# fperezgamonal/flownet2-tf

Hardware: AMD Instinct MI355X
Metric: forward pairs/sec at 512x384 (FlowNet2) (higher is better)
Workload: dtype f16x2 (split fp16 hi+lo operands, 3 fp16 MFMAs per product, fp32 accumulate); 1 GPU; FlowNet2 forward, batch=4 synthetic 512x384 pairs per GPU, seeded synthetic weights; pairs_per_gpu=4, parallelism=dp1 (no collective)

## Files before the change

flownet2-tf_amd/csrc/conv2.hip:

```cpp
#include "conv_common.h"

#include <type_traits>
#include <algorithm>
#include <utility>

#ifndef FN2_X2_ORDER
#define FN2_X2_ORDER 0
#endif
#ifndef FN2_CONV_ABLATE
#define FN2_CONV_ABLATE 0
#endif
#ifndef FN2_SETPRIO
#define FN2_SETPRIO 1
#endif

namespace fn2 {

typedef __attribute__((address_space(3))) void* lptr_t;

constexpr unsigned kOobOffset = 0x80000000u;

typedef int v4i_t __attribute__((ext_vector_type(4)));
typedef unsigned u32x4_t __attribute__((ext_vector_type(4)));

// ... 606 lines not shown
      const int m = m0 + wp * TPN * 32 + b * 16 + r16;
      if (m >= p.M) continue;
      const int n = m / (p.OH * p.OW);
      const int rem = m - n * (p.OH * p.OW);
      const int oy = rem / p.OW, ox = rem - oy * p.OW;
      const size_t opix = ((size_t)n * p.out_H + (oy * osc + oy_off)) * p.out_W + (ox * osc + ox_off);
      OutT* po = out16 + opix * p.out_cs + p.out_c0;
#pragma unroll
      for (int a = 0; a < TCN * 2; ++a) {
        const int co = c0 + wc * TCN * 32 + (a >> 1) * 32 + 16 * (g16 & 1) + 8 * (a & 1) + 4 * (g16 >> 1);
        if (slab != nullptr) {
          if (co < p.ws_cs)
            *reinterpret_cast<float4*>(slab + opix * p.ws_cs + co) =
                make_float4(acc16[a][b][0], acc16[a][b][1], acc16[a][b][2], acc16[a][b][3]);
          continue;
        }
        float v[4];
#pragma unroll
        for (int j = 0; j < 4; ++j) {
          float x = acc16[a][b][j] * p.out_scale + ((p.bias != nullptr && co + j < p.Cout) ? p.bias[co + j] : 0.f);
          if constexpr (sizeof(OutT) == 4) {
            if (p.accum && co + j < p.Cout) x += load_elem<OutT>(po + co + j);
            if (co + j < p.Cout) x = act_grad<OutT>(p, out16, po + co + j, co + j, x);
          }
          if (p.act == FN2_ACT_LEAKY) x = leaky(x);
          v[j] = x;
        }
        if (p.vec_ok && co + 3 < p.Cout) store_vec<OutT, 4>(po + co, v);
        else
#pragma unroll
          for (int j = 0; j < 4; ++j)
            if (co + j < p.Cout) store_elem<OutT>(po + co + j, v[j]);
      }
    }
    return;
  }

  OutT* out = reinterpret_cast<OutT*>(p.out);
  constexpr int WCOLS = TCN * 32, RS = WCOLS + 4, WROWS = 32 * TPN;
  constexpr int WTW = WROWS * RS + WROWS;
  constexpr bool kLdsT = (KG > 1 ? 4 : 2) * WTW * 4 <= KG * ROWS * 128;
  if constexpr (FEED && !kLdsT) { if (feeder) return; }
  float* const tl = reinterpret_cast<float*>(KG > 1 ? ep1 : (wave < 2 ? lds0_all : ep1)) + (KG > 1 ? wave : (wave & 1)) * WTW;
  constexpr int CPR = WCOLS / 4, RPI = 64 / CPR;
  static_assert(!SLAB || WREG, "SLAB is a specialisation of the WREG instantiations");
  if ((SLAB || !WREG) && p.splitk > 1) {
    float* slab = p.ws + (size_t)split * p.N * p.out_H * p.out_W * p.ws_cs;
    if constexpr (kLdsT) {
      if constexpr (STAGES >= 3) __syncthreads();
      if constexpr (FEED) { if (feeder) return; }
      int* rowoff = reinterpret_cast<int*>(tl + WROWS * RS);
#pragma unroll
      for (int tp = 0; tp < TPN; ++tp) {
        const int m = m0 + wp * TPN * 32 + tp * 32 + fr;
        const int mm = m < p.M ? m : 0;
        const int n = mm / (p.OH * p.OW);
        const int rem = mm - n * (p.OH * p.OW);
        const int oy = rem / p.OW, ox = rem - oy * p.OW;
        if (fh == 0) rowoff[tp * 32 + fr] = m < p.M ? (int)((((size_t)n * p.out_H + (oy * osc + oy_off)) * p.out_W + (ox * osc + ox_off)) * p.ws_cs) : -1;
#pragma unroll
        for (int tc = 0; tc < TCN; ++tc)
#pragma unroll
          for (int q = 0; q < 4; ++q)
            *reinterpret_cast<float4*>(tl + (tp * 32 + fr) * RS + tc * 32 + fh * 16 + q * 4) =
                make_float4(acc[tc][tp][4 * q], acc[tc][tp][4 * q + 1], acc[tc][tp][4 * q + 2], acc[tc][tp][4 * q + 3]);
      }
      const int rr = lane / CPR, ch = lane - rr * CPR;
      const int co = c0 + wc * WCOLS + ch * 4;
#pragma unroll
      for (int i = 0; i < WROWS / RPI; ++i) {
        const int row = i * RPI + rr;
        const float4 v = *reinterpret_cast<const float4*>(tl + row * RS + ch * 4);
        const int off = rowoff[row];
        if (off >= 0 && co < p.ws_cs) *reinterpret_cast<float4*>(slab + (size_t)off + co) = v;
      }
      return;
    }
#pragma unroll
    for (int tp = 0; tp < TPN; ++tp) {
      const int m = m0 + wp * TPN * 32 + tp * 32 + fr;
      if (m >= p.M) continue;
      const int n = m / (p.OH * p.OW);
      const int rem = m - n * (p.OH * p.OW);
      const int oy = rem / p.OW, ox = rem - oy * p.OW;
      float* po = slab + (((size_t)n * p.out_H + (oy * osc + oy_off)) * p.out_W + (ox * osc + ox_off)) * p.ws_cs;
#pragma unroll
      for (int tc = 0; tc < TCN; ++tc)
#pragma unroll
        for (int q = 0; q < 4; ++q) {
          const int co = c0 + wc * TCN * 32 + tc * 32 + fh * 16 + q * 4;
          if (co < p.ws_cs)
            *reinterpret_cast<float4*>(po + co) = make_float4(acc[tc][tp][4 * q], acc[tc][tp][4 * q + 1],
                                                              acc[tc][tp][4 * q + 2], acc[tc][tp][4 * q + 3]);
        }
    }
    return;
  }
  if constexpr (SLAB) return;
  const bool vec16 = (p.out_cs % 8 == 0) && (p.out_c0 % 8 == 0);
  const bool wide = kLdsT && sizeof(OutT) == 4 && vec16 && c0 + wc * WCOLS + WCOLS <= p.Cout && !(p.dbg & 4194304);
  int* const rowoff = reinterpret_cast<int*>(tl + WROWS * RS);
  if constexpr (STAGES >= 3 && kLdsT) __syncthreads();
  if constexpr (FEED) { if (feeder) return; }
#pragma unroll
  for (int tc = 0; tc < TCN; ++tc) {
    const int cout_base = c0 + wc * TCN * 32 + tc * 32 + fh * 16;
    float bias[16];
#pragma unroll
    for (int q = 0; q < 16; ++q) bias[q] = (p.bias != nullptr && cout_base + q < p.Cout) ? p.bias[cout_base + q] : 0.f;
#pragma unroll
    for (int tp = 0; tp < TPN; ++tp) {
      const int m = m0 + wp * TPN * 32 + tp * 32 + fr;
      if (wide && tc == 0 && fh == 0) rowoff[tp * 32 + fr] = m < p.M ? 0 : -1;
      if (m >= p.M) continue;
      const int n = m / (p.OH * p.OW);
      const int rem = m - n * (p.OH * p.OW);
      const int oy = rem / p.OW, ox = rem - oy * p.OW;
      const size_t opix = (((size_t)n * p.out_H + (oy * osc + oy_off)) * p.out_W + (ox * osc + ox_off));
      OutT* po = out + opix * p.out_cs + p.out_c0 + cout_base;
      float v[16];
#pragma unroll
      for (int q = 0; q < 16; ++q) v[q] = acc[tc][tp][q] * p.out_scale + bias[q];
      accum_act_grad16<OutT>(p, out, po, cout_base, vec16 && cout_base + 15 < p.Cout, v);
      if (p.act == FN2_ACT_LEAKY) {
#pragma unroll
        for (int q = 0; q < 16; ++q) v[q] = leaky(v[q]);
      }
      if (wide) {
        if (tc == 0 && fh == 0) rowoff[tp * 32 + fr] = (int)opix;
        store16<OutT>(reinterpret_cast<OutT*>(tl + (tp * 32 + fr) * RS + tc * 32 + fh * 16), v);
      } else if (vec16 && cout_base + 15 < p.Cout) {
        store16<OutT>(po, v);
      } else {
#pragma unroll
        for (int q = 0; q < 16; ++q)
          if (cout_base + q < p.Cout) store_elem<OutT>(po + q, v[q]);
      }
    }
  }
  if (wide) {
    const int rr = lane / CPR, ch = lane - rr * CPR;
    OutT* ob = out + p.out_c0 + c0 + wc * WCOLS + ch * 4;
#pragma unroll
    for (int i = 0; i < WROWS / RPI; ++i) {
      const int row = i * RPI + rr;
      const uint4 v = *reinterpret_cast<const uint4*>(tl + row * RS + ch * 4);
      const int opix = rowoff[row];
      if (opix >= 0) *reinterpret_cast<uint4*>(ob + (size_t)opix * p.out_cs) = v;
    }
  }
#endif
}

template <typename OutT, int WC, int WP, int TCN, int TPN, int KW>
__global__ void __launch_bounds__(256) conv_halo_kernel(const ConvArgs p) {
#if defined(__HIP_DEVICE_COMPILE__)
  using T = x2_t;
  constexpr int ESZ = 4;
  constexpr int BC = WC * TCN * 32, BP = WP * TPN * 32;
  static_assert(WC * WP == 4, "4 waves per block");
  constexpr int NWI = BC / 32;
  constexpr int BROWS = BP + 8;
  constexpr int NBP = BROWS / 8;
  constexpr int NBW = (NBP + 3) / 4;
  __shared__ uint4 ldsA[2][BC * 8];
  __shared__ uint4 ldsB[2][BROWS * 8];

  const int tid = threadIdx.x, lane = tid & 63;
  const int wave = __builtin_amdgcn_readfirstlane(tid >> 6);
  const int wc = wave / WP, wp = wave % WP;

  int pad_y = p.pad, pad_x = p.pad, oy_off = 0, ox_off = 0, osc = 1;
  const T* wgt = reinterpret_cast<const T*>(p.wgt);
  const int phase = blockIdx.z;
  const unsigned wrow_bytes = (unsigned)p.ksteps * 128u;
  if (p.merged) {
    pad_y = phase ? p.ph_pad1 : p.ph_pad0; pad_x = 1; oy_off = phase; ox_off = 0; osc = 2;
    wgt += (size_t)phase * p.cout_pad * (wrow_bytes / ESZ);
  } else if (p.deconv) {
    const int a = phase >> 1, b = phase & 1;
    pad_y = a ? p.ph_pad1 : p.ph_pad0; pad_x = b ? p.ph_pad1 : p.ph_pad0; oy_off = a; ox_off = b; osc = 2;
    wgt += (size_t)phase * p.cout_pad * (wrow_bytes / ESZ);
  }
  int bx = blockIdx.x, by = blockIdx.y;
  {
    const int NT = gridDim.x * gridDim.y, L = blockIdx.x + gridDim.x * blockIdx.y;
    const int xcd = L & 7, chunk = NT >> 3, rem = NT & 7;
    const int Lp = xcd * chunk + min(xcd, rem) + (L >> 3);
    bx = Lp / (int)gridDim.y;
    by = Lp - bx * (int)gridDim.y;
  }
  const int m0 = bx * BP, c0 = by * BC;
  const int tn = m0 / (p.OH * p.OW);
  const int trem = m0 - tn * (p.OH * p.OW);
  const int toy = trem / p.OW, tox = trem - toy * p.OW;
  const int iy_base = toy - pad_y, ix_base = tox - pad_x;

  const v4i_t rsrc_w = make_rsrc(wgt, (int)(p.cout_pad * wrow_bytes));
  const v4i_t rsrc_x = make_rsrc(p.in, p.in_bytes);
  const int lrow = lane >> 3, lphys = lane & 7;
  unsigned woff[NWI];
#pragma unroll
  for (int j = 0; j < NWI; ++j) {
    const int row = wave * (BC / 4) + j * 8 + lrow;
    woff[j] = (unsigned)(c0 + row) * wrow_bytes + (unsigned)((lphys ^ ((row >> 1) & 7)) * 16);
  }
  int boff[NBW];
  bool bok[NBW];
#pragma unroll
  for (int j = 0; j < NBW; ++j) {
    const int q = wave + 4 * j;
    const int e = q * 8 + lrow;
    const int ix = ix_base + e;
    bok[j] = q < NBP && e < BP + KW - 1 && ix >= 0 && ix < p.W;
    boff[j] = (((tn * p.H + iy_base) * p.W + ix) * p.in_cs + p.in_c0) * ESZ + (lphys ^ ((e >> 1) & 7)) * 16;
  }
  const int spt = p.cin_chunks >> 3;
  const int nsup = spt * p.KH;
  auto issue_B = [&](int sup, uint4* lds) {
    const int sc = sup / p.KH, ky = sup - sc * p.KH;
    const bool yok = (unsigned)(iy_base + ky) < (unsigned)p.H;
    const int toff = (ky * p.W * p.in_cs) * ESZ + sc * 128;
#pragma unroll
    for (int j = 0; j < NBW; ++j) {
      const int q = wave + 4 * j;
      if (q < NBP) dma16(rsrc_x, &lds[q * 64], (bok[j] && yok) ? (unsigned)(boff[j] + toff) : kOobOffset, 0);
    }
  };
  auto issue_A = [&](int sup, int kx, uint4* lds) {
    const int sc = sup / p.KH, ky = sup - sc * p.KH;
    const int soff = ((ky * KW + kx) * spt + sc) * 128;
#pragma unroll
    for (int j = 0; j < NWI; ++j) dma16(rsrc_w, &lds[(wave * (BC / 4) + j * 8) * 8], woff[j], soff);
  };

  const int fr = lane & 31, fh = lane >> 5, fsw = (fr >> 1) & 7;
  f32x16 acc[TCN][TPN];
#pragma unroll
  for (int tc = 0; tc < TCN; ++tc)
#pragma unroll
    for (int tp = 0; tp < TPN; ++tp)
#pragma unroll
      for (int q = 0; q < 16; ++q) acc[tc][tp][q] = 0.f;

  auto compute = [&](const uint4* la, const uint4* lb, int kx) {
#if FN2_SETPRIO
    __builtin_amdgcn_s_setprio(1);
#endif
    const uint4* A = &la[(wc * TCN * 32 + fr) * 8];
#pragma unroll
    for (int q = 0; q < 2; ++q) {
      const int chh = (4 * q + 2 * fh) ^ fsw, chl = (4 * q + 2 * fh + 1) ^ fsw;
      uint4 ah[TCN], al[TCN], bh[TPN], bl[TPN];
#pragma unroll
      for (int t = 0; t < TCN; ++t) { ah[t] = A[t * 32 * 8 + chh]; al[t] = A[t * 32 * 8 + chl]; }
#pragma unroll
      for (int t = 0; t < TPN; ++t) {
        const int rb = wp * TPN * 32 + t * 32 + fr + kx, sw = (rb >> 1) & 7;
        bh[t] = lb[rb * 8 + ((4 * q + 2 * fh) ^ sw)];
        bl[t] = lb[rb * 8 + ((4 * q + 2 * fh + 1) ^ sw)];
      }
#pragma unroll
      for (int tc = 0; tc < TCN; ++tc)
#pragma unroll
        for (int tp = 0; tp < TPN; ++tp) {
          acc[tc][tp] = mfma_32x32x16<f16_t>(al[tc], bh[tp], acc[tc][tp]);
          acc[tc][tp] = mfma_32x32x16<f16_t>(ah[tc], bl[tp], acc[tc][tp]);
          acc[tc][tp] = mfma_32x32x16<f16_t>(ah[tc], bh[tp], acc[tc][tp]);
        }
    }
#if FN2_SETPRIO
    __builtin_amdgcn_s_setprio(0);
#endif
  };

  issue_B(0, ldsB[0]);
  issue_A(0, 0, ldsA[0]);
  asm volatile("s_waitcnt vmcnt(0)" ::: "memory");
  __syncthreads();
  int abuf = 0;
  for (int sup = 0; sup < nsup; ++sup) {
#pragma unroll
    for (int kx = 0; kx < KW; ++kx) {
      if (kx + 1 < KW) issue_A(sup, kx + 1, ldsA[abuf ^ 1]);
      else if (sup + 1 < nsup) issue_A(sup + 1, 0, ldsA[abuf ^ 1]);
      if (kx == 0 && sup + 1 < nsup) issue_B(sup + 1, ldsB[(sup + 1) & 1]);
      compute(ldsA[abuf], ldsB[sup & 1], kx);
      asm volatile("s_waitcnt vmcnt(0)" ::: "memory");
      __syncthreads();
      abuf ^= 1;
    }
  }

  OutT* out = reinterpret_cast<OutT*>(p.out);
  const bool vec16 = (p.out_cs % 8 == 0) && (p.out_c0 % 8 == 0);
  constexpr int ERS = 36;
  static_assert(sizeof(ldsA) >= 4 * 32 * ERS * 4 || sizeof(ldsB) >= 4 * 32 * ERS * 4, "epilogue tiles fit a stage array");
  float* const etl = reinterpret_cast<float*>(sizeof(ldsA) >= 4 * 32 * ERS * 4 ? &ldsA[0][0] : &ldsB[0][0]) + wave * (32 * ERS);
#pragma unroll
  for (int tc = 0; tc < TCN; ++tc) {
    int cout_base = c0 + wc * TCN * 32 + tc * 32 + fh * 16;
    int bsel = 0;
    if (p.merged) { bsel = cout_base / p.Cout; cout_base -= bsel * p.Cout; if (bsel > 1) continue; }
    float bias[16];
#pragma unroll
    for (int q = 0; q < 16; ++q) bias[q] = (p.bias != nullptr && cout_base + q < p.Cout) ? p.bias[cout_base + q] : 0.f;
#pragma unroll
    for (int tp = 0; tp < TPN; ++tp) {
      const int ox = tox + wp * TPN * 32 + tp * 32 + fr;
      OutT* po = out + (((size_t)tn * p.out_H + (toy * osc + oy_off)) * p.out_W + (ox * osc + ox_off + bsel)) * p.out_cs +
                 p.out_c0 + cout_base;
      float v[16];
#pragma unroll
      for (int q = 0; q < 16; ++q) v[q] = acc[tc][tp][q] * p.out_scale + bias[q];
      accum_act_grad16<OutT>(p, out, po, cout_base, vec16 && cout_base + 15 < p.Cout, v);
      if (p.act == FN2_ACT_LEAKY) {
#pragma unroll
        for (int q = 0; q < 16; ++q) v[q] = leaky(v[q]);
      }
      if (sizeof(OutT) == 4 && vec16 && !p.merged && c0 + wc * TCN * 32 + tc * 32 + 32 <= p.Cout && !(p.dbg & 4194304)) {
        store16<OutT>(reinterpret_cast<OutT*>(etl + fr * ERS + fh * 16), v);
        const int rr = lane >> 3, ch = lane & 7;
        const int ox0 = tox + wp * TPN * 32 + tp * 32;
        OutT* ob = out + (((size_t)tn * p.out_H + (toy * osc + oy_off)) * p.out_W + (ox0 * osc + ox_off)) * p.out_cs +
                   p.out_c0 + c0 + wc * TCN * 32 + tc * 32 + ch * 4;
#pragma unroll
        for (int i = 0; i < 4; ++i) {
          const int row = i * 8 + rr;
          *reinterpret_cast<uint4*>(ob + (size_t)row * osc * p.out_cs) = *reinterpret_cast<const uint4*>(etl + row * ERS + ch * 4);
        }
      } else if (vec16 && cout_base + 15 < p.Cout) {
        store16<OutT>(po, v);
      } else {
#pragma unroll
        for (int q = 0; q < 16; ++q)
          if (cout_base + q < p.Cout) store_elem<OutT>(po + q, v[q]);
      }
      if (p.merged && p.up_src != nullptr && cout_base == 0 && ox < p.OW) {
        const int uy = toy * osc + oy_off, ux = ox * osc + ox_off + bsel;
        const int H2 = p.out_H >> 1, W2 = p.out_W >> 1;
        const int a = uy & 1, b = ux & 1, y = uy >> 1, x = ux >> 1;
        float r0 = p.up_bias ? p.up_bias[0] : 0.f, r1 = p.up_bias ? p.up_bias[1] : 0.f;
#pragma unroll
        for (int ty = 0; ty < 2; ++ty) {
          const int iy = y - 1 + a + ty, ky = 3 - a - 2 * ty;
          if (iy < 0 || iy >= H2) continue;
#pragma unroll
          for (int tx = 0; tx < 2; ++tx) {
            const int ix = x - 1 + b + tx, kx = 3 - b - 2 * tx;
            if (ix < 0 || ix >= W2) continue;
            const float2 sv = *reinterpret_cast<const float2*>(p.up_src + (((long)tn * H2 + iy) * W2 + ix) * 2);
            const float* ww = p.up_w + (ky * 4 + kx) * 4;
            r0 += sv.x * ww[0] + sv.y * ww[1];
            r1 += sv.x * ww[2] + sv.y * ww[3];
          }
        }
        OutT* pu = out + (((size_t)tn * p.out_H + uy) * p.out_W + ux) * p.out_cs + p.up_c0;
        store_elem<OutT>(pu, r0);
        store_elem<OutT>(pu + 1, r1);
      }
    }
  }
#endif
}

template <typename OutT, int NST>
__global__ void __launch_bounds__(256) conv_stem_kernel(const ConvArgs p, const int ntiles) {
#if defined(__HIP_DEVICE_COMPILE__)
  using T = x2_t;
  constexpr int ESZ = 4;
  constexpr int BC = 64, BP = 128, TCN = 2;
  __shared__ uint4 ldsA[NST][BC * 8];
  __shared__ uint4 ldsB[2][NST][BP * 8];
  const int tid = threadIdx.x, lane = tid & 63;
  const int wave = __builtin_amdgcn_readfirstlane(tid >> 6);
  const unsigned wrow_bytes = (unsigned)p.ksteps * 128u;
  const v4i_t rsrc_w = make_rsrc(p.wgt, (int)(p.cout_pad * wrow_bytes));
  const v4i_t rsrc_x = make_rsrc(p.in, p.in_bytes);
  const int lrow = lane >> 3, lphys = lane & 7;
  const int spt = p.cin_chunks >> 3;
#pragma unroll
  for (int st = 0; st < NST; ++st) {
    const int sc = st / p.KH, ky = st - sc * p.KH;
#pragma unroll
    for (int j = 0; j < 2; ++j) {
      const int row = wave * 16 + j * 8 + lrow;
      const unsigned woff = (unsigned)row * wrow_bytes + (unsigned)((lphys ^ ((row >> 1) & 7)) * 16);
      dma16(rsrc_w, &ldsA[st][(wave * 16 + j * 8) * 8], woff, (ky * spt + sc) * 128);
    }
  }
  auto issue_B = [&](int tile, int buf) {
#pragma unroll
    for (int j = 0; j < 4; ++j) {
      const int row = wave * 32 + j * 8 + lrow;
      const int m = tile * BP + row;
      const bool v = m < p.M && tile < ntiles;
      const int mm = v ? m : 0;
      const int n = mm / (p.OH * p.OW);
      const int rem = mm - n * (p.OH * p.OW);
      const int oy = rem / p.OW, ox = rem - oy * p.OW;
      const int roff = (((n * p.H + oy * p.stride) * p.W + ox * p.stride) * p.in_cs + p.in_c0) * ESZ +
                       (lphys ^ ((row >> 1) & 7)) * 16;
#pragma unroll
      for (int st = 0; st < NST; ++st) {
        const int sc = st / p.KH, ky = st - sc * p.KH;
        const int toff = (ky * p.W * p.in_cs) * ESZ + sc * 128;
        dma16(rsrc_x, &ldsB[buf][st][(wave * 32 + j * 8) * 8], v ? (unsigned)(roff + toff) : kOobOffset, 0);
      }
    }
  };
  const int fr = lane & 31, fh = lane >> 5, fsw = (fr >> 1) & 7;
  OutT* out = reinterpret_cast<OutT*>(p.out);
  const bool vec16 = (p.out_cs % 8 == 0) && (p.out_c0 % 8 == 0);
  float bias[TCN][16];
#pragma unroll
  for (int tc = 0; tc < TCN; ++tc)
#pragma unroll
    for (int q = 0; q < 16; ++q) {
      const int co = tc * 32 + fh * 16 + q;
      bias[tc][q] = (p.bias != nullptr && co < p.Cout) ? p.bias[co] : 0.f;
    }

  int tile = blockIdx.x, cur = 0;
  issue_B(tile, 0);
  asm volatile("s_waitcnt vmcnt(0)" ::: "memory");
  __syncthreads();
  for (; tile < ntiles; tile += gridDim.x, cur ^= 1) {
    issue_B(tile + gridDim.x, cur ^ 1);
    f32x16 acc[TCN];
#pragma unroll
    for (int tc = 0; tc < TCN; ++tc)
#pragma unroll
      for (int q = 0; q < 16; ++q) acc[tc][q] = 0.f;
#if FN2_SETPRIO
    __builtin_amdgcn_s_setprio(1);
#endif
#pragma unroll
    for (int st = 0; st < NST; ++st) {
      const uint4* A = &ldsA[st][fr * 8];
      const uint4* B = &ldsB[cur][st][(wave * 32 + fr) * 8];
#pragma unroll
      for (int q = 0; q < 2; ++q) {
        const int chh = (4 * q + 2 * fh) ^ fsw, chl = (4 * q + 2 * fh + 1) ^ fsw;
        const uint4 bh = B[chh], bl = B[chl];
#pragma unroll
        for (int tc = 0; tc < TCN; ++tc) {
          const uint4 ah = A[tc * 32 * 8 + chh], al = A[tc * 32 * 8 + chl];
          acc[tc] = mfma_32x32x16<f16_t>(al, bh, acc[tc]);
          acc[tc] = mfma_32x32x16<f16_t>(ah, bl, acc[tc]);
          acc[tc] = mfma_32x32x16<f16_t>(ah, bh, acc[tc]);
        }
      }
    }
#if FN2_SETPRIO
    __builtin_amdgcn_s_setprio(0);
#endif
    const int m = tile * BP + wave * 32 + fr;
    if (m < p.M) {
      const int n = m / (p.OH * p.OW);
      const int rem = m - n * (p.OH * p.OW);
      const int oy = rem / p.OW, ox = rem - oy * p.OW;
#pragma unroll
      for (int tc = 0; tc < TCN; ++tc) {
        const int cout_base = tc * 32 + fh * 16;
        OutT* po = out + (((size_t)n * p.out_H + oy) * p.out_W + ox) * p.out_cs + p.out_c0 + cout_base;
        float v[16];
#pragma unroll
        for (int q = 0; q < 16; ++q) {
          float x = acc[tc][q] * p.out_scale + bias[tc][q];
          if (p.act == FN2_ACT_LEAKY) x = leaky(x);
          v[q] = x;
        }
        if (vec16 && cout_base + 15 < p.Cout) {
          store16<OutT>(po, v);
        } else {
#pragma unroll
          for (int q = 0; q < 16; ++q)
            if (cout_base + q < p.Cout) store_elem<OutT>(po + q, v[q]);
        }
      }
    }
    asm volatile("s_waitcnt vmcnt(0)" ::: "memory");
    __syncthreads();
  }
#endif
}

template <int CPR>
__global__ void __launch_bounds__(512) head5_strip_kernel(const ConvArgs p) {
#if defined(__HIP_DEVICE_COMPILE__)
  constexpr int RD = 4, CL = 3, NL = CPR * CL;
  constexpr int TS = 68;
  __shared__ uint4 ldsW[NL][64 * 8];
  __shared__ uint4 ldsX[RD][CL][64 * 8];
  __shared__ float T[50 * TS];
  __shared__ float accr[5 * 64 * 2];
  const int tid = threadIdx.x, lane = tid & 63;
  const int wave = __builtin_amdgcn_readfirstlane(tid >> 6);
  const bool feeder = wave >= 4;
  const int w4 = wave & 3;
  const int wc = w4 >> 1, wp = w4 & 1;
  const int H = p.OH, W = p.OW;
  const int nstrip = p.h5_tx, nseg = p.h5_ty, R = p.h5_rows;
  const int b = blockIdx.x;
  const int sx = b % nstrip, sg = (b / nstrip) % nseg, n = b / (nstrip * nseg);
  const int x0 = sx * 60 - 2;
  const int y0 = sg * R, y1 = min(H, y0 + R);
  const int r0 = max(0, y0 - 2), r1 = min(H - 1, y1 + 1);
  const int nch = (r1 - r0 + 1) * CPR;
  const float bias_o[2] = {p.bias ? p.bias[0] : 0.f, p.bias ? p.bias[1] : 0.f};
  const unsigned wrow_bytes = (unsigned)p.ksteps * 128u;
  const v4i_t rsrc_w = make_rsrc(p.wgt, (int)(p.cout_pad * wrow_bytes));
  const v4i_t rsrc_x = make_rsrc(p.in, p.in_bytes);
// ... 171 lines not shown
  }
  const int nl = p.cin_chunks >> 3;
  const int ngroups = (p.KH_KW_hint * p.in_cs + 7) >> 3;
  auto issue_B = [&](int ky, uint4* lds) {
    const int toff = ky * p.W * p.in_cs * 4;
#pragma unroll
    for (int j = 0; j < NBW; ++j) {
      const int q = wave + 4 * j;
      if (q < npieces) dma16(rsrc_x, &lds[q * 64], boff[j] == kOobOffset ? kOobOffset : boff[j] + (unsigned)toff, 0);
    }
  };
  auto issue_A = [&](int ky, int l, uint4* lds) {
    const int soff = (ky * nl + l) * 128;
#pragma unroll
    for (int j = 0; j < 2; ++j) dma16(rsrc_w, &lds[(wave * 16 + j * 8) * 8], woff[j], soff);
  };

  const int fr = lane & 31, fh = lane >> 5, fsw = (fr >> 1) & 7;
  const int pslot = (wave * 32 + fr) * p.stride * SPP;
  f32x16 acc[TCN];
#pragma unroll
  for (int tc = 0; tc < TCN; ++tc)
#pragma unroll
    for (int q = 0; q < 16; ++q) acc[tc][q] = 0.f;

  issue_B(0, ldsB[0]);
  issue_A(0, 0, ldsA[0]);
  asm volatile("s_waitcnt vmcnt(0)" ::: "memory");
  __syncthreads();
  int abuf = 0;
  for (int ky = 0; ky < p.KH; ++ky) {
    const uint4* lb = ldsB[ky & 1];
    for (int l = 0; l < nl; ++l) {
      if (l + 1 < nl) issue_A(ky, l + 1, ldsA[abuf ^ 1]);
      else if (ky + 1 < p.KH) issue_A(ky + 1, 0, ldsA[abuf ^ 1]);
      if (l == 0 && ky + 1 < p.KH) issue_B(ky + 1, ldsB[(ky + 1) & 1]);
#if FN2_SETPRIO
      __builtin_amdgcn_s_setprio(1);
#endif
      const uint4* A = &ldsA[abuf][fr * 8];
#pragma unroll
      for (int q = 0; q < 2; ++q) {
        if (4 * l + 2 * q >= ngroups) continue;
        const int chh = (4 * q + 2 * fh) ^ fsw, chl = (4 * q + 2 * fh + 1) ^ fsw;
        const int g = 4 * l + 2 * q + fh;
        const int sh = pslot + 2 * g, sl = sh + 1;
        const uint4 bh = lb[sh ^ ((sh >> 4) & 15)], bl = lb[sl ^ ((sl >> 4) & 15)];
#pragma unroll
        for (int tc = 0; tc < TCN; ++tc) {
          const uint4 ah = A[tc * 32 * 8 + chh], al = A[tc * 32 * 8 + chl];
          acc[tc] = mfma_32x32x16<f16_t>(al, bh, acc[tc]);
          acc[tc] = mfma_32x32x16<f16_t>(ah, bl, acc[tc]);
          acc[tc] = mfma_32x32x16<f16_t>(ah, bh, acc[tc]);
        }
      }
#if FN2_SETPRIO
      __builtin_amdgcn_s_setprio(0);
#endif
      asm volatile("s_waitcnt vmcnt(0)" ::: "memory");
      __syncthreads();
      abuf ^= 1;
    }
  }

  OutT* out = reinterpret_cast<OutT*>(p.out);
  const bool vec16 = (p.out_cs % 8 == 0) && (p.out_c0 % 8 == 0);
  const int ox = tox + wave * 32 + fr;
  constexpr int ERS = 36;
  float* const tl = reinterpret_cast<float*>(&ldsB[0][0]) + wave * (32 * ERS);
  static_assert(4 * 32 * ERS * 4 <= (int)sizeof(ldsB), "epilogue tiles fit the segment buffers");
#pragma unroll
  for (int tc = 0; tc < TCN; ++tc) {
    const int cout_base = c0 + tc * 32 + fh * 16;
    OutT* po = out + (((size_t)tn * p.out_H + toy) * p.out_W + ox) * p.out_cs + p.out_c0 + cout_base;
    float v[16];
#pragma unroll
    for (int q = 0; q < 16; ++q) {
      float x = acc[tc][q] * p.out_scale + ((p.bias != nullptr && cout_base + q < p.Cout) ? p.bias[cout_base + q] : 0.f);
      if (p.act == FN2_ACT_LEAKY) x = leaky(x);
      v[q] = x;
    }
    if (sizeof(OutT) == 4 && vec16 && c0 + tc * 32 + 32 <= p.Cout && !(p.dbg & 4194304)) {
      store16<OutT>(reinterpret_cast<OutT*>(tl + fr * ERS + fh * 16), v);
      const int rr = lane >> 3, ch = lane & 7;
      OutT* ob = out + (((size_t)tn * p.out_H + toy) * p.out_W + tox + wave * 32) * p.out_cs + p.out_c0 + c0 + tc * 32 + ch * 4;
#pragma unroll
      for (int i = 0; i < 4; ++i) {
        const int row = i * 8 + rr;
        *reinterpret_cast<uint4*>(ob + (size_t)row * p.out_cs) = *reinterpret_cast<const uint4*>(tl + row * ERS + ch * 4);
      }
    } else if (vec16 && cout_base + 15 < p.Cout) {
      store16<OutT>(po, v);
    } else {
#pragma unroll
      for (int q = 0; q < 16; ++q)
        if (cout_base + q < p.Cout) store_elem<OutT>(po + q, v[q]);
    }
  }
#endif
}

template <typename OutT>
static bool launch_rowrun(const ConvArgs& a, int tile, int phases, hipStream_t s) {
  if ((a.dbg & 65536) || tile != 64 || phases != 1 || a.deconv || a.KW != 1 || a.KH_KW_hint < 1 || a.splitk != 1 || a.accum || a.wfrag)
    return false;
  if (a.OW % 128 != 0 || (a.in_cs != 8 && a.in_cs != 16)) return false;
  const int spp = a.in_cs / 4;
  const int nl = a.cin_chunks >> 3;
  const int max_slot = 127 * a.stride * spp + 2 * (4 * nl - 1) + 1;
  const int npieces = max_slot / 64 + 1;
  if (npieces > (spp == 4 ? 17 : 9)) return false;
  dim3 grid(a.M / 128, a.cout_pad / 64, 1), block(256);
  if (conv_name_sink().buf) {
    snprintf(conv_name_sink().buf, conv_name_sink().cap, "conv_rowrun_kernel<%s, %d>", is_x2<OutT>::value ? "fn2::x2_t" : "float", spp);
    return true;
  }
  if (spp == 4) hipLaunchKernelGGL((conv_rowrun_kernel<OutT, 4>), grid, block, 0, s, a, npieces);
  else hipLaunchKernelGGL((conv_rowrun_kernel<OutT, 2>), grid, block, 0, s, a, npieces);
  return true;
}

template <typename OutT>
static bool launch_stem(const ConvArgs& a, int tile, int phases, hipStream_t s) {
  if ((a.dbg & 8192) || tile != 64 || phases != 1 || a.deconv || a.KW != 1 || a.splitk != 1 || a.accum ||
      a.ksteps < 1 || a.ksteps > 4 || a.cout_pad != 64)
    return false;
  const int ntiles = cdiv(a.M, 128);
  if (ntiles < 512) return false;
  const char* e = getenv("FN2_STEM_BLOCKS");
  const int blocks = std::min(ntiles, e ? atoi(e) : 256);
  if (conv_name_sink().buf) {
    snprintf(conv_name_sink().buf, conv_name_sink().cap, "conv_stem_kernel<%s, %d>",
             is_x2<OutT>::value ? "fn2::x2_t" : "float", a.ksteps);
    return true;
  }
  switch (a.ksteps) {
    case 1: hipLaunchKernelGGL((conv_stem_kernel<OutT, 1>), dim3(blocks), dim3(256), 0, s, a, ntiles); break;
    case 2: hipLaunchKernelGGL((conv_stem_kernel<OutT, 2>), dim3(blocks), dim3(256), 0, s, a, ntiles); break;
    case 3: hipLaunchKernelGGL((conv_stem_kernel<OutT, 3>), dim3(blocks), dim3(256), 0, s, a, ntiles); break;
    default: hipLaunchKernelGGL((conv_stem_kernel<OutT, 4>), dim3(blocks), dim3(256), 0, s, a, ntiles); break;
  }
  return true;
}

template <typename OutT>
static bool launch_halo(const ConvArgs& a, int tile, int phases, hipStream_t s) {
  if (((a.dbg & 2048) && !a.merged) || a.stride != 1 || a.splitk != 1 || a.kg != 1 || !a.bp64 || a.wfrag || (a.KW != 2 && a.KW != 3)) return false;
  if (a.deconv && (a.kh_ph[0] != a.KH || a.kh_ph[1] != a.KH || a.kw_ph[0] != a.KW || a.kw_ph[1] != a.KW)) return false;
  if (tile == 128 && a.bp64 == 2 && !(a.dbg & 4096)) return false;
  if (a.bp64 == 3) return false;
  const int bp = tile == 128 ? 64 : 128;
  if (a.OW % bp != 0 || a.M % bp != 0) return false;
  dim3 block(256);
#define FN2_HALO(GY, ...)                                                                         \
  do {                                                                                            \
    dim3 grid(a.M / bp, GY, phases);                                                              \
    if (conv_name_sink().buf)                                                                     \
      snprintf(conv_name_sink().buf, conv_name_sink().cap, "conv_halo_kernel<%s, %s, %d>",       \
               is_x2<OutT>::value ? "fn2::x2_t" : "float", #__VA_ARGS__, a.KW);                    \
    else if (a.KW == 3) hipLaunchKernelGGL((conv_halo_kernel<OutT, __VA_ARGS__, 3>), grid, block, 0, s, a); \
    else hipLaunchKernelGGL((conv_halo_kernel<OutT, __VA_ARGS__, 2>), grid, block, 0, s, a);      \
  } while (0)
  if (tile == 128) FN2_HALO(a.cout_pad / 128, 2, 2, 2, 1);
  else if (tile == 64) FN2_HALO(a.cout_pad / 64, 1, 4, 2, 1);
  else FN2_HALO(a.cout_pad / 32, 1, 4, 1, 1);
#undef FN2_HALO
  return true;
}

ConvNameSink& conv_name_sink() {
  static thread_local ConvNameSink sink{nullptr, 0};
  return sink;
}

template <typename T, typename OutT>
static int launch2(const ConvArgs& a, int tile, int phases, hipStream_t s) {
  const int z = phases * a.splitk;
  const long blocks64 = (long)cdiv(a.M, 64) * (a.cout_pad / 128) * z;
  const char* e_m16 = getenv("FN2_M16_MIN");
  const bool m16 = is_x2<T>::value && !(a.dbg & 512) &&
                   ((a.dbg & 1024) || (e_m16 && tile == 128 && a.bp64 == 1 && a.kg == 1 && a.splitk == 1 &&
                                       blocks64 >= atoi(e_m16)));
#define FN2_LAUNCH2(GX, GY, THREADS, ...)                                                              \
  do {                                                                                                 \
    dim3 grid(GX, GY, z);                                                                              \
    if (conv_name_sink().buf)                                                                          \
      snprintf(conv_name_sink().buf, conv_name_sink().cap, "conv_igemm2_kernel<%s, %s, %s, %s>", type_name<T>(), \
               type_name<OutT>(), #__VA_ARGS__, m16 ? "true" : "false");                              \
    else if (m16) hipLaunchKernelGGL((conv_igemm2_kernel<T, OutT, __VA_ARGS__, is_x2<T>::value>), grid, dim3(THREADS), 0, s, a); \
    else hipLaunchKernelGGL((conv_igemm2_kernel<T, OutT, __VA_ARGS__, false>), grid, dim3(THREADS), 0, s, a);            \
  } while (0)
  if (a.wfrag) {
    if constexpr (is_x2<T>::value) {
      if (tile == 64) {
        dim3 grid(cdiv(a.M, 128), a.cout_pad / 64, z);
        if (conv_name_sink().buf)
          snprintf(conv_name_sink().buf, conv_name_sink().cap, "conv_igemm2_kernel<%s, %s, 2, 2, 1, 2, 2, 1, false, true, %s>",
                   type_name<T>(), type_name<OutT>(), a.splitk > 1 ? "true" : "false");
        else if (a.splitk > 1)
          hipLaunchKernelGGL((conv_igemm2_kernel<T, OutT, 2, 2, 1, 2, 2, 1, false, true, true>), grid, dim3(256), 0, s, a);
        else
          hipLaunchKernelGGL((conv_igemm2_kernel<T, OutT, 2, 2, 1, 2, 2, 1, false, true, false>), grid, dim3(256), 0, s, a);
      } else {
        dim3 grid(cdiv(a.M, 64), a.cout_pad / 128, z);
        const bool slab = a.splitk > 1;
        ConvArgs ah = a;
        if (a.fh_M > 0 && slab && !conv_name_sink().buf) {
          const char* e = getenv("FN2_FH_BLOCKS");
          const long per_z = (long)grid.x * grid.y;
          const long want = std::min<long>(a.fh_M, e ? atoi(e) : 1024);
          ah.fh_z0 = z;
          grid.z = z + (unsigned)std::max<long>(1, (want + per_z - 1) / per_z);
        } else {
          ah.fh_M = 0;
        }
        const ConvArgs& a = ah;
        const char* e_feed = getenv("FN2_WREG_FEED");
        const int feed = e_feed ? atoi(e_feed) : 1;
        if (conv_name_sink().buf)
          snprintf(conv_name_sink().buf, conv_name_sink().cap, "conv_igemm2_kernel<%s, %s, 4, 1, 1, 2, %d, 1, false, true, %s%s>",
                   type_name<T>(), type_name<OutT>(), a.wfrag == 2 ? 3 : 2, slab ? "true" : "false",
                   (a.wfrag == 2 && (slab ? feed >= 2 : feed >= 1)) ? ", false, true" : "");
        else if (a.wfrag == 2 && slab && feed >= 2)
          hipLaunchKernelGGL((conv_igemm2_kernel<T, OutT, 4, 1, 1, 2, 3, 1, false, true, true, false, true>), grid, dim3(512), 0, s, a);
        else if (a.wfrag == 2 && slab)
          hipLaunchKernelGGL((conv_igemm2_kernel<T, OutT, 4, 1, 1, 2, 3, 1, false, true, true>), grid, dim3(256), 0, s, a);
        else if (a.wfrag == 2 && feed >= 1)
          hipLaunchKernelGGL((conv_igemm2_kernel<T, OutT, 4, 1, 1, 2, 3, 1, false, true, false, false, true>), grid, dim3(512), 0, s, a);
        else if (a.wfrag == 2)
          hipLaunchKernelGGL((conv_igemm2_kernel<T, OutT, 4, 1, 1, 2, 3, 1, false, true, false>), grid, dim3(256), 0, s, a);
        else if (slab)
          hipLaunchKernelGGL((conv_igemm2_kernel<T, OutT, 4, 1, 1, 2, 2, 1, false, true, true>), grid, dim3(256), 0, s, a);
        else
          hipLaunchKernelGGL((conv_igemm2_kernel<T, OutT, 4, 1, 1, 2, 2, 1, false, true, false>), grid, dim3(256), 0, s, a);
      }
    } else {
      return fail(FN2_ERR_UNSUPPORTED, "conv fast path: fragment-order weights are split fp16 only");
    }
  } else if (tile == 128 && a.bp64 && a.kg == 3) FN2_LAUNCH2(cdiv(a.M, 64), a.cout_pad / 128, 768, 2, 2, 2, 1, 2, 3);
  else if (tile == 128 && a.bp64 && a.kg == 2) FN2_LAUNCH2(cdiv(a.M, 64), a.cout_pad / 128, 512, 2, 2, 2, 1, 2, 2);
  else if (tile == 128 && a.bp64 == 3) FN2_LAUNCH2(cdiv(a.M, 64), a.cout_pad / 128, 256, 2, 2, 2, 1, 6, 1);
  else if (tile == 128 && a.bp64 == 2) FN2_LAUNCH2(cdiv(a.M, 64), a.cout_pad / 128, 256, 2, 2, 2, 1, 3, 1);
  else if (tile == 128 && a.bp64) FN2_LAUNCH2(cdiv(a.M, 64), a.cout_pad / 128, 256, 2, 2, 2, 1, 2, 1);
  else if (tile == 128) FN2_LAUNCH2(cdiv(a.M, 128), a.cout_pad / 128, 256, 2, 2, 2, 2, 2, 1);
  else if (tile == 64 && a.bp64) FN2_LAUNCH2(cdiv(a.M, 128), a.cout_pad / 64, 256, 1, 4, 2, 1, 2, 1);
  else if (tile == 64) FN2_LAUNCH2(cdiv(a.M, 256), a.cout_pad / 64, 256, 1, 4, 2, 2, 2, 1);
  else if (a.bp64) FN2_LAUNCH2(cdiv(a.M, 128), a.cout_pad / 32, 256, 1, 4, 1, 1, 2, 1);
  else FN2_LAUNCH2(cdiv(a.M, 256), a.cout_pad / 32, 256, 1, 4, 1, 2, 2, 1);
#undef FN2_LAUNCH2
  return conv_launched("conv_igemm2");
}

int launch_head5_strip(const ConvArgs& a, int blocks, hipStream_t s) {
  if (a.ksteps != 3 && a.ksteps != 6) return fail(FN2_ERR_UNSUPPORTED, "flow_head5 strip form: %d channel lines (3 or 6)", a.ksteps);
  if (conv_name_sink().buf) FN2_CONV_NAME("head5_strip_kernel<%d>", a.ksteps / 3);
  else if (a.ksteps == 3) hipLaunchKernelGGL((head5_strip_kernel<1>), dim3(blocks), dim3(512), 0, s, a);
  else hipLaunchKernelGGL((head5_strip_kernel<2>), dim3(blocks), dim3(512), 0, s, a);
  return conv_launched("flow_head5_strip");
}

int launch_head5(const ConvArgs& a, int blocks, hipStream_t s) {
  if (conv_name_sink().buf)
    FN2_CONV_NAME("conv_igemm2_kernel<fn2::x2_t, float, 1, 4, 2, 2, 2, 1, false, false, false, true>");
  else
    hipLaunchKernelGGL((conv_igemm2_kernel<x2_t, float, 1, 4, 2, 2, 2, 1, false, false, false, true>), dim3(blocks, 1, 1), dim3(256), 0,
                       s, a);
  return conv_launched("flow_head5");
}

bool conv_fast_ok(int in_dtype, int cin_pad, int cout) {
  const int esz = dtype_size(in_dtype);
  return cout > 2 && (cin_pad * esz) % 128 == 0;
}

int launch_conv_fast(const ConvArgs& a, int in_dtype, int out_dtype, int tile, int phases, hipStream_t s) {
  if (tile != 128 && tile != 64 && tile != 32) return fail(FN2_ERR_UNSUPPORTED, "conv fast path: cout tile %d", tile);
  if (in_dtype == FN2_F32) return launch2<float, float>(a, tile, phases, s);
  if (in_dtype == FN2_BF16) {
    if (out_dtype == FN2_BF16) return launch2<bf16_t, bf16_t>(a, tile, phases, s);
    return launch2<bf16_t, float>(a, tile, phases, s);
  }
  if (in_dtype == FN2_F16) {
    if (out_dtype == FN2_F16) return launch2<f16_t, f16_t>(a, tile, phases, s);
    return launch2<f16_t, float>(a, tile, phases, s);
  }
  if (out_dtype == FN2_F16X2) {
    if (launch_rowrun<x2_t>(a, tile, phases, s)) return conv_launched("conv_rowrun");
    if (launch_stem<x2_t>(a, tile, phases, s)) return conv_launched("conv_stem");
    if (launch_halo<x2_t>(a, tile, phases, s)) return conv_launched("conv_halo");
    if (a.merged) return fail(FN2_ERR_UNSUPPORTED, "conv2d kind 5: needs the halo kernel (input width a multiple of 128, no split-K)");
    return launch2<x2_t, x2_t>(a, tile, phases, s);
  }
  if (launch_halo<float>(a, tile, phases, s)) return conv_launched("conv_halo");
  if (a.merged) return fail(FN2_ERR_UNSUPPORTED, "conv2d kind 5: needs the halo kernel (input width a multiple of 128, no split-K)");
  return launch2<x2_t, float>(a, tile, phases, s);
}

}
```

Before: 1101 pairs/s.

## Add per-phase-tap halo kernel for merged deconv with 16x16 MFMA path

Adds a PT template variant of the halo conv kernel for merged (phase-decomposed) deconvolutions. Each wave loads and multiplies only the two horizontal taps that are nonzero for its phase instead of the full 3-wide window, which removes wasted weight DMA and MFMAs. For narrow outputs (Cout 16) a dedicated 16x16x32 MFMA path is added, with an LDS-staged vectorized epilogue and a fused upsampled-flow store written as paired fp16 hi/lo. The flow-upsample code moves into a shared helper. The cost is more template variants and more complex indexing and swizzle logic, which carries some correctness risk.

```diff
diff --git a/flownet2-tf_amd/csrc/conv2.hip b/flownet2-tf_amd/csrc/conv2.hip
--- a/flownet2-tf_amd/csrc/conv2.hip
+++ b/flownet2-tf_amd/csrc/conv2.hip
@@ -782,18 +782,58 @@
 #endif
 }
 
-template <typename OutT, int WC, int WP, int TCN, int TPN, int KW>
+template <typename OutT>
+__device__ __forceinline__ void halo_upflow_pixel(const ConvArgs& p, OutT* out, int n, int uy, int ux) {
+  const int H2 = p.out_H >> 1, W2 = p.out_W >> 1;
+  const int a = uy & 1, b = ux & 1, y = uy >> 1, x = ux >> 1;
+  float r0 = p.up_bias ? p.up_bias[0] : 0.f, r1 = p.up_bias ? p.up_bias[1] : 0.f;
+#pragma unroll
+  for (int ty = 0; ty < 2; ++ty) {
+    const int iy = y - 1 + a + ty, ky = 3 - a - 2 * ty;
+    if (iy < 0 || iy >= H2) continue;
+#pragma unroll
+    for (int tx = 0; tx < 2; ++tx) {
+      const int ix = x - 1 + b + tx, kx = 3 - b - 2 * tx;
+      if (ix < 0 || ix >= W2) continue;
+      const float2 sv = *reinterpret_cast<const float2*>(p.up_src + (((long)n * H2 + iy) * W2 + ix) * 2);
+      const float* ww = p.up_w + (ky * 4 + kx) * 4;
+      r0 += sv.x * ww[0] + sv.y * ww[1];
+      r1 += sv.x * ww[2] + sv.y * ww[3];
+    }
+  }
+  OutT* pu = out + (((size_t)n * p.out_H + uy) * p.out_W + ux) * p.out_cs + p.up_c0;
+  if ((p.up_c0 | p.out_cs) & 1) {
+    store_elem<OutT>(pu, r0);
+    store_elem<OutT>(pu + 1, r1);
+  } else if constexpr (is_x2<OutT>::value) {
+    typedef __attribute__((ext_vector_type(2))) _Float16 h2;
+    const size_t addr = reinterpret_cast<size_t>(pu);
+    _Float16* g = reinterpret_cast<_Float16*>(addr & ~size_t(31)) + ((addr & 31) >> 2);
+    const _Float16 h0 = (_Float16)r0, h1 = (_Float16)r1;
+    *reinterpret_cast<h2*>(g) = h2{h0, h1};
+    *reinterpret_cast<h2*>(g + 8) = h2{(_Float16)(r0 - (float)h0), (_Float16)(r1 - (float)h1)};
+  } else {
+    const float rr[2] = {r0, r1};
+    store_vec<OutT, 2>(pu, rr);
+  }
+}
+
+template <typename OutT, int WC, int WP, int TCN, int TPN, int KW, int PT = 0>
 __global__ void __launch_bounds__(256) conv_halo_kernel(const ConvArgs p) {
 #if defined(__HIP_DEVICE_COMPILE__)
   using T = x2_t;
   constexpr int ESZ = 4;
+  constexpr bool kPT = PT != 0;
+  constexpr bool kP16 = kPT && TCN == 1;
+  static_assert(!kPT || (KW == 3 && WC == 1 && WP == 4 && TPN == 1 && TCN <= 2), "per-phase taps: the 2 x 3 window of kind 5");
   constexpr int BC = WC * TCN * 32, BP = WP * TPN * 32;
   static_assert(WC * WP == 4, "4 waves per block");
   constexpr int NWI = BC / 32;
   constexpr int BROWS = BP + 8;
   constexpr int NBP = BROWS / 8;
   constexpr int NBW = (NBP + 3) / 4;
-  __shared__ uint4 ldsA[2][BC * 8];
+  constexpr int AROWS = kP16 ? 64 : BC;
+  __shared__ uint4 ldsA[2][AROWS * 8];
   __shared__ uint4 ldsB[2][BROWS * 8];
 
   const int tid = threadIdx.x, lane = tid & 63;
@@ -860,9 +900,123 @@
   auto issue_A = [&](int sup, int kx, uint4* lds) {
     const int sc = sup / p.KH, ky = sup - sc * p.KH;
     const int soff = ((ky * KW + kx) * spt + sc) * 128;
+    if (kPT && kx != wave / 2 && kx != wave / 2 + 1) return;
 #pragma unroll
     for (int j = 0; j < NWI; ++j) dma16(rsrc_w, &lds[(wave * (BC / 4) + j * 8) * 8], woff[j], soff);
   };
+
+  if constexpr (kP16) {
+    const int r16 = lane & 15, g16 = lane >> 4;
+    const int pr = r16 ^ ((r16 & 8) >> 1);
+    const int ch = 2 * (((g16 & 1) << 1) | (g16 >> 1));
+    const int wb = wave >> 1, wkx = (wave >> 1) + (wave & 1);
+    unsigned woff16[2];
+#pragma unroll
+    for (int j = 0; j < 2; ++j) {
+      const int fr16 = j * 8 + lrow;
+      const int co = fr16 ^ ((fr16 & 8) >> 1);
+      const int prow = (co & 3) + 8 * (co >> 2) + 4 * wb;
+      const int row = wave * 16 + fr16;
+      woff16[j] = (unsigned)(c0 + prow) * wrow_bytes + (unsigned)((lphys ^ ((row >> 1) & 7)) * 16);
+    }
+    auto issue_A16 = [&](int sup, uint4* lds) {
+      const int sc = sup / p.KH, ky = sup - sc * p.KH;
+      const int soff = ((ky * KW + wkx) * spt + sc) * 128;
+#pragma unroll
+      for (int j = 0; j < 2; ++j) dma16(rsrc_w, &lds[(wave * 16 + j * 8) * 8], woff16[j], soff);
+    };
+    f32x4 acc16[2][2];
+#pragma unroll
+    for (int b = 0; b < 2; ++b)
+#pragma unroll
+      for (int sp = 0; sp < 2; ++sp) acc16[b][sp] = f32x4{0.f, 0.f, 0.f, 0.f};
+    auto compute16 = [&](const uint4* la, const uint4* lb) {
+#if FN2_SETPRIO
+      __builtin_amdgcn_s_setprio(1);
+#endif
+      uint4 bh[KW][2], bl[KW][2];
+#pragma unroll
+      for (int kx = 0; kx < KW; ++kx)
+#pragma unroll
+        for (int sp = 0; sp < 2; ++sp) {
+          const int rb = wave * 32 + sp * 16 + pr + kx, sw = (rb >> 1) & 7;
+          bh[kx][sp] = lb[rb * 8 + (ch ^ sw)];
+          bl[kx][sp] = lb[rb * 8 + ((ch + 1) ^ sw)];
+        }
+#pragma unroll
+      for (int c = 0; c < 4; ++c) {
+        const int b = c >> 1, kx = (c >> 1) + (c & 1);
+        const int ra = c * 16 + pr, sw = (ra >> 1) & 7;
+        const uint4 ah = la[ra * 8 + (ch ^ sw)], al = la[ra * 8 + ((ch + 1) ^ sw)];
+#pragma unroll
+        for (int sp = 0; sp < 2; ++sp) {
+          acc16[b][sp] = mfma_16x16x32<f16_t>(al, bh[kx][sp], acc16[b][sp]);
+          acc16[b][sp] = mfma_16x16x32<f16_t>(ah, bl[kx][sp], acc16[b][sp]);
+          acc16[b][sp] = mfma_16x16x32<f16_t>(ah, bh[kx][sp], acc16[b][sp]);
+        }
+      }
+#if FN2_SETPRIO
+      __builtin_amdgcn_s_setprio(0);
+#endif
+    };
+    issue_B(0, ldsB[0]);
+    issue_A16(0, ldsA[0]);
+    asm volatile("s_waitcnt vmcnt(0)" ::: "memory");
+    __syncthreads();
+    for (int sup = 0; sup < nsup; ++sup) {
+      if (sup + 1 < nsup) {
+        issue_A16(sup + 1, ldsA[(sup + 1) & 1]);
+        issue_B(sup + 1, ldsB[(sup + 1) & 1]);
+      }
+      compute16(ldsA[sup & 1], ldsB[sup & 1]);
+      asm volatile("s_waitcnt vmcnt(0)" ::: "memory");
+      __syncthreads();
+    }
+    OutT* out = reinterpret_cast<OutT*>(p.out);
+    constexpr int ERB = 80;
+    static_assert(sizeof(ldsB) >= 4 * 64 * ERB, "epilogue tiles fit the pixel stage buffers");
+    char* const etl = reinterpret_cast<char*>(&ldsB[0][0]) + wave * (64 * ERB);
+    float bias[4];
+#pragma unroll
+    for (int i = 0; i < 4; ++i) bias[i] = p.bias != nullptr ? p.bias[4 * g16 + i] : 0.f;
+#pragma unroll
+    for (int b = 0; b < 2; ++b)
+#pragma unroll
+      for (int sp = 0; sp < 2; ++sp) {
+        float v[4];
+#pragma unroll
+        for (int i = 0; i < 4; ++i) {
+          v[i] = acc16[b][sp][i] * p.out_scale + bias[i];
+          if (p.act == FN2_ACT_LEAKY) v[i] = leaky(v[i]);
+        }
+        char* row = etl + (2 * (sp * 16 + pr) + b) * ERB;
+        if constexpr (is_x2<OutT>::value) {
+          typedef __attribute__((ext_vector_type(4))) _Float16 h4;
+          h4 h, l;
+#pragma unroll
+          for (int i = 0; i < 4; ++i) {
+            h[i] = (_Float16)v[i];
+            l[i] = (_Float16)(v[i] - (float)h[i]);
+          }
+          char* grp = row + (g16 >> 1) * 32 + (g16 & 1) * 8;
+          *reinterpret_cast<h4*>(grp) = h;
+          *reinterpret_cast<h4*>(grp + 16) = l;
+        } else {
+          *reinterpret_cast<float4*>(row + g16 * 16) = make_float4(v[0], v[1], v[2], v[3]);
+        }
+      }
+    asm volatile("s_waitcnt lgkmcnt(0)" ::: "memory");
+    const int uy = toy * 2 + phase, ux0 = (tox + wave * 32) * 2;
+    char* const ob = reinterpret_cast<char*>(out + (((size_t)tn * p.out_H + uy) * p.out_W + ux0) * p.out_cs + p.out_c0);
+#pragma unroll
+    for (int i = 0; i < 4; ++i) {
+      const int R = i * 16 + (lane >> 2), part = lane & 3;
+      *reinterpret_cast<uint4*>(ob + (size_t)R * p.out_cs * sizeof(OutT) + part * 16) =
+          *reinterpret_cast<const uint4*>(etl + R * ERB + part * 16);
+    }
+    if (p.up_src != nullptr) halo_upflow_pixel<OutT>(p, out, tn, uy, ux0 + lane);
+    return;
+  }
 
   const int fr = lane & 31, fh = lane >> 5, fsw = (fr >> 1) & 7;
   f32x16 acc[TCN][TPN];
@@ -891,13 +1045,15 @@
         bl[t] = lb[rb * 8 + ((4 * q + 2 * fh + 1) ^ sw)];
       }
 #pragma unroll
-      for (int tc = 0; tc < TCN; ++tc)
+      for (int tc = 0; tc < TCN; ++tc) {
+        if (kPT && kx != tc && kx != tc + 1) continue;
 #pragma unroll
         for (int tp = 0; tp < TPN; ++tp) {
           acc[tc][tp] = mfma_32x32x16<f16_t>(al[tc], bh[tp], acc[tc][tp]);
           acc[tc][tp] = mfma_32x32x16<f16_t>(ah[tc], bl[tp], acc[tc][tp]);
           acc[tc][tp] = mfma_32x32x16<f16_t>(ah[tc], bh[tp], acc[tc][tp]);
         }
+      }
     }
 #if FN2_SETPRIO
     __builtin_amdgcn_s_setprio(0);
@@ -966,29 +1122,8 @@
         for (int q = 0; q < 16; ++q)
           if (cout_base + q < p.Cout) store_elem<OutT>(po + q, v[q]);
       }
-      if (p.merged && p.up_src != nullptr && cout_base == 0 && ox < p.OW) {
-        const int uy = toy * osc + oy_off, ux = ox * osc + ox_off + bsel;
-        const int H2 = p.out_H >> 1, W2 = p.out_W >> 1;
-        const int a = uy & 1, b = ux & 1, y = uy >> 1, x = ux >> 1;
-        float r0 = p.up_bias ? p.up_bias[0] : 0.f, r1 = p.up_bias ? p.up_bias[1] : 0.f;
-#pragma unroll
-        for (int ty = 0; ty < 2; ++ty) {
-          const int iy = y - 1 + a + ty, ky = 3 - a - 2 * ty;
-          if (iy < 0 || iy >= H2) continue;
-#pragma unroll
-          for (int tx = 0; tx < 2; ++tx) {
-            const int ix = x - 1 + b + tx, kx = 3 - b - 2 * tx;
-            if (ix < 0 || ix >= W2) continue;
-            const float2 sv = *reinterpret_cast<const float2*>(p.up_src + (((long)tn * H2 + iy) * W2 + ix) * 2);
-            const float* ww = p.up_w + (ky * 4 + kx) * 4;
-            r0 += sv.x * ww[0] + sv.y * ww[1];
-            r1 += sv.x * ww[2] + sv.y * ww[3];
-          }
-        }
-        OutT* pu = out + (((size_t)tn * p.out_H + uy) * p.out_W + ux) * p.out_cs + p.up_c0;
-        store_elem<OutT>(pu, r0);
-        store_elem<OutT>(pu + 1, r1);
-      }
+      if (p.merged && p.up_src != nullptr && cout_base == 0 && ox < p.OW)
+        halo_upflow_pixel<OutT>(p, out, tn, toy * osc + oy_off, ox * osc + ox_off + bsel);
     }
   }
 #endif
@@ -1466,7 +1601,17 @@
   const int bp = tile == 128 ? 64 : 128;
   if (a.OW % bp != 0 || a.M % bp != 0) return false;
   dim3 block(256);
-#define FN2_HALO(GY, ...)                                                                         \
+  if (a.merged && !(a.dbg & 128) && tile == 32 &&
+      (a.Cout == 32 || (!a.accum && a.mask_y == nullptr && a.out_cs % 8 == 0 && a.out_c0 % 8 == 0))) {
+    dim3 grid(a.M / bp, 1, phases);
+    if (conv_name_sink().buf)
+      snprintf(conv_name_sink().buf, conv_name_sink().cap, "conv_halo_kernel<%s, 1, 4, %d, 1, 3, 1>",
+               is_x2<OutT>::value ? "fn2::x2_t" : "float", a.Cout / 16);
+    else if (a.Cout == 32) hipLaunchKernelGGL((conv_halo_kernel<OutT, 1, 4, 2, 1, 3, 1>), grid, block, 0, s, a);
+    else hipLaunchKernelGGL((conv_halo_kernel<OutT, 1, 4, 1, 1, 3, 1>), grid, block, 0, s, a);
+    return true;
+  }
+#define FN2_HALO(GY, ...)                                                                        \
   do {                                                                                            \
     dim3 grid(a.M / bp, GY, phases);                                                              \
     if (conv_name_sink().buf)                                                                     \
```

After: 1115 pairs/s (median of 6 runs). +1.3%, better.
